# foubari/ratio_guided_Multimodal_FM

Measured on AMD Instinct MI355X. Metric: paired images/sec (MNIST32+SVHN, 100 Euler steps), higher is better.
Workload: dtype f32; 1 GPU; MNIST32 (1x32x32) + SVHN (3x32x32) pair, mc_feng guidance 0.5, 100 Euler steps, N_mc=256, batch 512 per GPU (BASELINE configs[2]; configs[3] at 8 GPUs); global_batch=512, parallelism=rows sharded over 1 rank(s); all_gather(MC set) + gather(outputs), step=one full sampling call (MC pre-phase + ratio + guided Euler loop + gather)

## Files before the change

### include/rgfm.h

```cpp
#ifndef RGFM_H_
#define RGFM_H_

#include <stddef.h>
#include <stdint.h>

#ifdef __cplusplus
extern "C" {
#endif

#define RGFM_ABI_VERSION 3

#define RGFM_OK 0
#define RGFM_EINVAL (-1)
#define RGFM_ENOMEM (-2)
#define RGFM_EHIP (-3)
#define RGFM_ENODEVICE (-4)

#define RGFM_MAX_LEVELS 4

typedef void* rgfm_stream_t;

typedef struct rgfm_unet_desc {
  int32_t in_channels;
  int32_t img_size;
// ... 1 lines not shown
  int32_t num_levels;
  int32_t channel_mult[RGFM_MAX_LEVELS];
  int32_t num_res_blocks;
} rgfm_unet_desc;

typedef struct rgfm_unet rgfm_unet;

int rgfm_unet_param_floats(const rgfm_unet_desc* desc, size_t* n_floats);

int rgfm_unet_create(const rgfm_unet_desc* desc, const float* params_dev, size_t n_floats,
                     rgfm_stream_t stream, rgfm_unet** out);
void rgfm_unet_destroy(rgfm_unet* h);

int rgfm_unet_workspace_bytes(const rgfm_unet* h, int batch, size_t* bytes);

int rgfm_unet_forward(rgfm_unet* h, const float* x, const float* t_dev, int t_count, float* v_out,
                      int batch, void* ws, size_t ws_bytes, rgfm_stream_t stream);

int rgfm_unet_set_trace(rgfm_unet* h, int enable);
int rgfm_unet_time_embedding(rgfm_unet* h, const float* t_dev, int t_count, float* emb_out, void* ws,
                             size_t ws_bytes, rgfm_stream_t stream);
int rgfm_unet_num_activations(const rgfm_unet* h, int* n);
int rgfm_unet_p_handovers(const rgfm_unet* h, int* blocks);
int rgfm_unet_wino_convs(const rgfm_unet* h, int* convs);
#define RGFM_ROUTE_HX2D 0
#define RGFM_ROUTE_HX2W 1
#define RGFM_ROUTE_HX2S 2
#define RGFM_ROUTE_HX2C 3
#define RGFM_ROUTE_HX2Q 4
#define RGFM_ROUTE_HX2P 5
#define RGFM_ROUTE_HX2 6
#define RGFM_ROUTE_BX3 7
#define RGFM_ROUTE_F32 8
#define RGFM_ROUTE_COUNT 9
#define RGFM_ROUTE_T2 9
#define RGFM_ROUTE_SLOTS 10
int rgfm_unet_conv_routes(const rgfm_unet* h, int* counts, int n);
int rgfm_unet_activation_shape(const rgfm_unet* h, int index, int* channels, int* height, int* width);
int rgfm_unet_read_activation(rgfm_unet* h, int index, int batch, const void* ws, float* out_dev,
                              rgfm_stream_t stream);

int rgfm_unet_train_workspace_bytes(const rgfm_unet* h, int batch, size_t* bytes);
int rgfm_unet_forward_train(rgfm_unet* h, const float* x, const float* t_dev, int t_count, float* v_out, int batch,
                            float p_drop, uint64_t seed, void* ws, size_t ws_bytes, rgfm_stream_t stream);
int rgfm_unet_backward(rgfm_unet* h, const float* dv, float* dx_out, float* dparams_out, int batch, void* ws,
                       size_t ws_bytes, rgfm_stream_t stream);
// ... 239 lines not shown
```

### ratio_guided_multimodal_fm_amd/_lib.py

```python
import ctypes
import os

_HERE = os.path.dirname(os.path.abspath(__file__))
LIB_PATH = os.environ.get("RGFM_LIB") or os.path.join(_HERE, "csrc", "librgfm_hip.so")
ABI_VERSION = 3

_lib = None

c_void_p, c_int, c_size_t, c_double = ctypes.c_void_p, ctypes.c_int, ctypes.c_size_t, ctypes.c_double
c_int32, c_int64, c_uint64, c_float = ctypes.c_int32, ctypes.c_int64, ctypes.c_uint64, ctypes.c_float
P = ctypes.POINTER


class UNetDesc(ctypes.Structure):
    _fields_ = [("in_channels", c_int32), ("img_size", c_int32), ("model_channels", c_int32),
                ("num_levels", c_int32), ("channel_mult", c_int32 * 4), ("num_res_blocks", c_int32)]


class RatioDesc(ctypes.Structure):
    _fields_ = [("kind", c_int32), ("feature_dim", c_int32), ("hidden_dim", c_int32),
                ("loss_type", c_int32)]


class RatioFlexDesc(ctypes.Structure):
    _fields_ = [("feature_dim", c_int32), ("hidden_dim", c_int32), ("loss_type", c_int32),
                ("x_channels", c_int32), ("y_channels", c_int32), ("x_size", c_int32), ("y_size", c_int32)]


class FmNetDesc(ctypes.Structure):
    _fields_ = [("img_channels", c_int32), ("feature_dim", c_int32), ("time_emb_dim", c_int32)]


class ClfDesc(ctypes.Structure):
    _fields_ = [("kind", c_int32)]


SIGNATURES = {
    "rgfm_unet_param_floats": (c_int, [P(UNetDesc), P(c_size_t)]),
    "rgfm_unet_create": (c_int, [P(UNetDesc), c_void_p, c_size_t, c_void_p, P(c_void_p)]),
    "rgfm_unet_destroy": (None, [c_void_p]),
    "rgfm_unet_workspace_bytes": (c_int, [c_void_p, c_int, P(c_size_t)]),
    "rgfm_unet_forward": (c_int, [c_void_p, c_void_p, c_void_p, c_int, c_void_p, c_int, c_void_p,
                                  c_size_t, c_void_p]),
    "rgfm_unet_set_trace": (c_int, [c_void_p, c_int]),
    "rgfm_unet_p_handovers": (c_int, [c_void_p, P(c_int)]),
    "rgfm_unet_wino_convs": (c_int, [c_void_p, P(c_int)]),
    "rgfm_unet_conv_routes": (c_int, [c_void_p, P(c_int), c_int]),
    "rgfm_unet_time_embedding": (c_int, [c_void_p, c_void_p, c_int, c_void_p, c_void_p, c_size_t, c_void_p]),
    "rgfm_unet_num_activations": (c_int, [c_void_p, P(c_int)]),
    "rgfm_unet_activation_shape": (c_int, [c_void_p, c_int, P(c_int), P(c_int), P(c_int)]),
    "rgfm_unet_read_activation": (c_int, [c_void_p, c_int, c_int, c_void_p, c_void_p, c_void_p]),
    "rgfm_unet_train_workspace_bytes": (c_int, [c_void_p, c_int, P(c_size_t)]),
    "rgfm_unet_forward_train": (c_int, [c_void_p, c_void_p, c_void_p, c_int, c_void_p, c_int, c_float, c_uint64,
                                        c_void_p, c_size_t, c_void_p]),
    "rgfm_unet_backward": (c_int, [c_void_p, c_void_p, c_void_p, c_void_p, c_int, c_void_p, c_size_t, c_void_p]),
    "rgfm_unet_vjp": (c_int, [c_void_p, c_void_p, c_void_p, c_int, c_void_p, c_size_t, c_void_p]),
    "rgfm_unet_divergence_workspace_bytes": (c_int, [c_void_p, c_int, P(c_size_t)]),
    "rgfm_unet_divergence": (c_int, [c_void_p, c_void_p, c_void_p, c_int, c_void_p, c_int, c_void_p, c_void_p, c_int,
                                     c_void_p, c_size_t, c_void_p]),
    "rgfm_unet_log_prob_workspace_bytes": (c_int, [c_void_p, c_int, c_int, c_int, P(c_size_t)]),
    "rgfm_unet_log_prob": (c_int, [c_void_p, c_void_p, c_void_p, c_int, c_int, c_int, c_void_p, c_void_p, c_int,
                                   c_void_p, c_size_t, c_void_p]),
    "rgfm_unet_dropout_mask": (c_int, [c_void_p, c_int, c_uint64, c_float, c_int, c_void_p]),
    "rgfm_unet_update_params": (c_int, [c_void_p, c_void_p, c_size_t, c_void_p]),
    "rgfm_ratio_param_floats": (c_int, [P(RatioDesc), P(c_size_t)]),
    "rgfm_ratio_create": (c_int, [P(RatioDesc), c_void_p, c_size_t, c_void_p, P(c_void_p)]),
    "rgfm_ratio_flex_param_floats": (c_int, [P(RatioFlexDesc), P(c_size_t)]),
    "rgfm_ratio_flex_create": (c_int, [P(RatioFlexDesc), c_void_p, c_size_t, c_void_p, P(c_void_p)]),
# ... 150 lines not shown
```

### ratio_guided_multimodal_fm_amd/csrc/api_unet.cpp

```cpp
#include "rgfm_host.h"

extern "C" int rgfm_unet_param_floats(const rgfm_unet_desc* desc, size_t* n_floats) {
  int rc = check_desc(desc);
  if (rc) return rc;
  if (!n_floats) return fail(RGFM_EINVAL, "null output");
  *n_floats = plan_unet(*desc, nullptr);
  return RGFM_OK;
}

static int pack_weights(rgfm_unet* h, hipStream_t s) {
  std::vector<HxImage*> images;
  std::vector<NormGate> gates;
  std::vector<ConvW*> res_convs;
  for (auto* v : {&h->enc, &h->mid, &h->dec})
    for (ResW& r : *v) {
      res_convs.push_back(&r.c1), res_convs.push_back(&r.c2);
      if (r.has_skip) res_convs.push_back(&r.sk);
      gates.push_back({r.n1w, r.n1b, r.cin, &r.c1.hx}), gates.push_back({r.n2w, r.n2b, r.cout, &r.c2.hx});
    }
  for (ConvW* w : res_convs) pack_one(h, *w, CONV_S1, s), images.push_back(&w->hx);
  for (ConvW& w : h->down) {
    pack_one(h, w, CONV_S2, s), images.push_back(&w.hx);
    launch_pack_conv_hx2(h->params + w.w_raw, h->packedh + w.hx9.off, h->hq + 4 * w.hx9.hq, w.cout, w.cin, 9, CONV_S1, s);
    images.push_back(&w.hx9);
// ... 161 lines not shown
  }
  for (int i = 0; i < 4; ++i) t.push_back({ch, S});
  for (int l = d.num_levels - 1; l >= 0; --l) {
    const int oc = h->mc * d.channel_mult[l];
    for (int i = 0; i < d.num_res_blocks + 1; ++i) {
      t.push_back({oc, S});
      t.push_back({oc, S});
      ch = oc;
    }
    if (l > 0) {
      S *= 2;
      t.push_back({ch, S});
    }
  }
  t.push_back({d.in_channels, S});
}
}

extern "C" int rgfm_unet_p_handovers(const rgfm_unet* h, int* blocks) {
  if (!h || !blocks) return fail(RGFM_EINVAL, "null argument");
  *blocks = h->p_handovers;
  return RGFM_OK;
}
extern "C" int rgfm_unet_wino_convs(const rgfm_unet* h, int* convs) {
  if (!h || !convs) return fail(RGFM_EINVAL, "null argument");
  *convs = h->wino_convs;
  return RGFM_OK;
}
extern "C" int rgfm_unet_conv_routes(const rgfm_unet* h, int* counts, int n) {
  if (!h || !counts || n < 0) return fail(RGFM_EINVAL, "null argument or negative count");
  for (int i = 0; i < n && i < RGFM_ROUTE_SLOTS; ++i) counts[i] = h->routes[i];
  return RGFM_OK;
}

extern "C" int rgfm_unet_num_activations(const rgfm_unet* h, int* n) {
  if (!h || !n) return fail(RGFM_EINVAL, "null argument");
  std::vector<std::pair<int, int>> t;
  act_table(h, t);
  *n = (int)t.size();
  return RGFM_OK;
}

extern "C" int rgfm_unet_activation_shape(const rgfm_unet* h, int index, int* channels, int* height, int* width) {
  if (!h) return fail(RGFM_EINVAL, "null handle");
  std::vector<std::pair<int, int>> t;
  act_table(h, t);
// ... 18 lines not shown
```

### ratio_guided_multimodal_fm_amd/csrc/rgfm_host.h

```cpp
#pragma once
#include "../../include/rgfm.h"

#include <hip/hip_runtime.h>

#include <algorithm>
#include <cmath>
#include <cstdarg>
#include <cstdio>
#include <cstdlib>
#include <cstring>
#include <string>
#include <vector>

#include "rgfm_kernels.h"

using namespace rgfm;

inline thread_local std::string g_err;

inline int fail(int code, const char* fmt, ...) {
  char buf[512];
  va_list ap;
  va_start(ap, fmt);
  vsnprintf(buf, sizeof(buf), fmt, ap);
// ... 178 lines not shown
  bool has_skip = false;
  int temb_off = 0;
};

inline int nt32_of(int cout) { return (cout % 64 == 0) ? 2 : 1; }

inline bool on_gfx950() {
  int dev = 0;
  if (hipGetDevice(&dev) != hipSuccess) return false;
  hipDeviceProp_t p;
  if (hipGetDeviceProperties(&p, dev) != hipSuccess) return false;
  return strncmp(p.gcnArchName, "gfx950", 6) == 0;
}

enum { CONV_ARITH_HX2 = 0, CONV_ARITH_BX3 = 1, CONV_ARITH_F32 = 2 };
struct Modes {
  int conv = CONV_ARITH_HX2;
  bool overlap = true, fuse_fin = true, gn_consumer = true;
  bool pipelined = true;
  bool quad = true;
  bool c8 = true;
  bool s2 = true;
  bool pfmt = true;
  bool wino = false;
  bool up_t2 = true;
  bool rev_hx2 = true;
  bool prephase = true;
  bool graph = false;
};
inline thread_local Modes g_modes;
inline void refresh_modes() {
  Modes m;
  const char* e = getenv("RGFM_CONV");
  if (e && strcmp(e, "bx3") == 0) m.conv = CONV_ARITH_BX3;
  else if (e && strcmp(e, "f32") == 0) m.conv = CONV_ARITH_F32;
  e = getenv("RGFM_OVERLAP");
  m.overlap = !(e && e[0] == '0');
  e = getenv("RGFM_FUSE_FIN");
  m.fuse_fin = !(e && e[0] == '0');
  e = getenv("RGFM_GN");
  m.gn_consumer = !(e && strcmp(e, "table") == 0);
  e = getenv("RGFM_HX2P");
  m.pipelined = !(e && e[0] == '0');
  e = getenv("RGFM_HX2Q");
  m.quad = !(e && e[0] == '0');
  e = getenv("RGFM_HX2S");
  m.s2 = !(e && e[0] == '0');
  e = getenv("RGFM_HX2C");
  m.c8 = !(e && e[0] == '0');
  e = getenv("RGFM_HX2D");
  m.pfmt = !(e && e[0] == '0');
  g_conv_tuning.hx2d_cut = e && e[0] == '1' ? 1 : (e && e[0] == '2' ? 2 : 3);
  e = getenv("RGFM_WINO");
  m.wino = e && e[0] == '1';
  e = getenv("RGFM_UP_T2");
  m.up_t2 = !(e && e[0] == '0');
  e = getenv("RGFM_REV_HX2");
  m.rev_hx2 = !(e && e[0] == '0');
  e = getenv("RGFM_GRAPH");
  m.graph = e && e[0] == '1';
  e = getenv("RGFM_PREPHASE_PRIO");
  m.prephase = !(e && e[0] == '0');
  g_modes = m;
  e = getenv("RGFM_WINO_W32");
  g_conv_tuning.wino_w32 = e ? atoi(e) : 0;
  g_conv_tuning.s2_f32 = getenv("RGFM_S2_F32") != nullptr;
  g_conv_tuning.f32_simple = getenv("RGFM_CONV_SIMPLE") != nullptr;
}

struct ModeScope {
  int saved;
  explicit ModeScope(int handle_mode) : saved(g_modes.conv) {
    if (handle_mode >= 0) g_modes.conv = handle_mode;
  }
  ~ModeScope() { g_modes.conv = saved; }
// ... 9 lines not shown
  hipEvent_t pre_pace = nullptr;
  hipStream_t main = nullptr;
  hipEvent_t main_fork = nullptr, main_join = nullptr;
  hipEvent_t graph_done = nullptr;
  std::vector<std::pair<hipGraphExec_t, hipGraph_t>> graphs;
};
inline DevState g_dev[MAX_DEVICES];

inline DevState* cur_dev() {
  int dev = 0;
  if (hipGetDevice(&dev) != hipSuccess || dev < 0 || dev >= MAX_DEVICES) return nullptr;
  return g_dev[dev].init ? &g_dev[dev] : nullptr;
}

inline int ensure_init() {
  if (!on_gfx950()) return fail(RGFM_ENODEVICE, "librgfm_hip needs a gfx950 (MI355X) device; none is current");
  int dev = 0;
  HIP_TRY(hipGetDevice(&dev));
  if (dev < 0 || dev >= MAX_DEVICES) return fail(RGFM_EINVAL, "device ordinal %d out of range (max %d)", dev, MAX_DEVICES - 1);
  DevState& d = g_dev[dev];
  if (!d.init) {
    int rc = guid_apply_init();
    for (const ConvKernel& k : CONV_KERNELS) rc |= k.init();
    if (rc != 0) return fail(RGFM_EHIP, "hipFuncSetAttribute(MaxDynamicSharedMemorySize) failed");
    hipDeviceProp_t p;
    if (hipGetDeviceProperties(&p, dev) == hipSuccess) d.num_cus = p.multiProcessorCount;
    const char* e = getenv("RGFM_HX2P_HALF");
    g_conv_tuning.hx2p_half = e ? atoi(e) : d.num_cus;
    HIP_TRY(hipStreamCreateWithFlags(&d.side, hipStreamNonBlocking));
    HIP_TRY(hipMalloc(&d.zeros, 256));
    HIP_TRY(hipMemset(d.zeros, 0, 256));
    HIP_TRY(hipEventCreateWithFlags(&d.fork, hipEventDisableTiming));
    HIP_TRY(hipEventCreateWithFlags(&d.join, hipEventDisableTiming));
    HIP_TRY(hipEventCreateWithFlags(&d.graph_done, hipEventDisableTiming));
    HIP_TRY(hipStreamCreateWithFlags(&d.main, hipStreamNonBlocking));
    HIP_TRY(hipEventCreateWithFlags(&d.main_fork, hipEventDisableTiming));
    HIP_TRY(hipEventCreateWithFlags(&d.main_join, hipEventDisableTiming));
    HIP_TRY(hipEventCreateWithFlags(&d.pre_pace, hipEventDisableTiming));
    d.init = true;
  }
  return RGFM_OK;
}

inline bool hx2w_pays(const ConvArgs& c) {
  return c.wpkw != nullptr && c.C0 + c.C1 >= 128 && (!g_conv_tuning.wino_w32 || c.g.W == 32);
}
// ... 114 lines not shown
  if (hipMemcpyAsync(host.data(), st.params, host.size() * sizeof(float), hipMemcpyDeviceToHost, s) != hipSuccess ||
      hipStreamSynchronize(s) != hipSuccess)
    return fail(RGFM_EHIP, "reading the parameters back failed");
  for (const NormGate& g : gates)
    if (!norm_params_ok(host, g.gamma, g.beta, g.C)) g.image->ok = false;
  return RGFM_OK;
}


struct rgfm_unet : WeightStore {
  rgfm_unet_desc d;
  float* freqs = nullptr;
  TimeLinear* lin_dev = nullptr;
  float* wtmp = nullptr;
  int mc = 0, temb = 0, nlin = 0, temb_total = 0;
  size_t te0w, te0b, te2w, te2b, icw, icb, onw, onb, ocw, ocb;
  size_t ocw_pk = 0;
  std::vector<ResW> enc, mid, dec;
  std::vector<ConvW> down, up;
  int final_ch = 0;
  bool trace = false;
  int wino_convs = 0;
  int p_handovers = 0;
  int routes[RGFM_ROUTE_SLOTS] = {};
  struct Act {
    float* data;
    int C, S;
    bool nchw;
  };
  std::vector<Act> acts;
};


inline size_t plan_unet(const rgfm_unet_desc& d, rgfm_unet* h) {
  Planner P;
  Cursor& c = P.raw;
  const int mc = d.model_channels, temb = 4 * mc;
  std::vector<ResW> enc, mid, dec;
  std::vector<ConvW> down, up;
  int temb_off = 0;
  auto res = [&](int cin, int cout) {
    ResW r;
    r.cin = cin, r.cout = cout;
    r.n1w = c.take(cin), r.n1b = c.take(cin);
    r.c1 = P.conv(cin, cout, 9);
    r.tw = c.take((size_t)cout * temb), r.tb = c.take(cout);
// ... 91 lines not shown
inline void fill_hx2(ConvArgs& c, const WeightStore& st, const ConvW& w, const ConvW* sk) {
  if (!w.hx.usable() || (sk && !sk->hx.usable())) return;
  c.wpkh = st.packedh + w.hx.off, c.hq = st.hq + 4 * w.hx.hq, c.range_flag = st.range_flag;
  if (w.hx9.usable()) c.wpkh9 = st.packedh + w.hx9.off;
  if (w.wino.usable() && !sk) c.wpkw = st.packedh + w.wino.off, c.hqw = st.hq + 4 * w.wino.hq;
  if (sk) c.wskiph = st.packedh + sk->hx.off, c.hq_skip = st.hq + 4 * sk->hx.hq;
}

inline double conv_flops(int B, int HW, int cout, int kprod) { return 2.0 * B * HW * (double)cout * kprod; }

inline bool up_parts_match(int S) {
  const TileGeom gl = make_geom(S, S), gf = make_geom(2 * S, 2 * S);
  if (gf.nparts != 4 * gl.nparts || gf.nparts > 16) return false;
  for (int p = 0; p < gf.nparts; ++p)
    if (geom_part_count(gf, p) != geom_part_count(gl, p % gl.nparts)) return false;
  return true;
}

struct PendingConv {
  bool valid = false;
  ConvArgs c{};
  int mode = 0;
  double flops = 0.0;
};

inline void flush_conv(PendingConv& p, hipStream_t s, int* routes = nullptr) {
  if (!p.valid) return;
  p.valid = false;
  ProfScope ps(RGFM_KCLASS_CONV_MFMA, p.flops, s);
  launch_conv(p.c, p.mode, s, routes);
}

inline bool try_fuse_finalize(PendingConv& p, const float* first_data, const float* stats1, int C1, const float* gamma,
                       const float* beta, float* ab, unsigned* counter) {
  if (!g_modes.fuse_fin || !p.valid || !counter || p.c.out != first_data || !p.c.stats_out) return false;
  if (p.c.pin0) return false;
  if ((p.c.Cout + C1) % 8 != 0 || p.c.Cout + C1 < 32 || p.c.Cout + C1 > 256) return false;
  if (p.c.g.nparts * (p.mode == CONV_T2 ? 4 : 1) > 16) return false;
  p.c.fin_ab = ab, p.c.fin_counter = counter, p.c.fin_expected = conv_fin_expected(p.c, p.mode);
  p.c.fin_stats1 = stats1, p.c.fin_C1 = C1, p.c.fin_gamma = gamma, p.c.fin_beta = beta;
  return true;
}

inline bool try_consumer_gn(ConvArgs& c, int mode, const float* stats0, const float* stats1, int nparts0, const TileGeom& gg,
                     const float* gamma, const float* beta) {
  c.gn_stats0 = stats0, c.gn_stats1 = stats1, c.gn_gamma = gamma, c.gn_beta = beta, c.gn_nparts0 = nparts0, c.gn_g = gg;
  bool ok = false;
  if (g_modes.gn_consumer) {
    if (g_modes.conv == CONV_ARITH_HX2 && conv_hx2_supported(c, mode)) ok = conv_hx2_gn_supported(c, mode);
    else if (g_modes.conv != CONV_ARITH_F32) ok = conv_bx3_gn_supported(c, mode);
  }
  if (!ok) c.gn_stats0 = c.gn_stats1 = c.gn_gamma = c.gn_beta = nullptr;
  return ok;
}

struct NormRef {
  size_t gamma, beta;
};
// ... 65 lines not shown
    c.out = o.data, c.stats_out = o.stats;
    c.B = B, c.Cout = w.cout;
    c.g = make_geom(So, So);
    c.halo_px = mode == CONV_S2 ? c.g.spt * (2 * c.g.th + 1) * (2 * c.g.W + 1) : c.g.spt * (c.g.th + 2) * (c.g.W + 2);
    const int kprod = 9 * w.cin + (res_mode == 2 ? sk->cin : 0);
    fill_hx2(c, *h, w, res_mode == 2 ? sk : nullptr);
    if (g_modes.conv == CONV_ARITH_HX2) c.range_flag = h->range_flag, c.small_check = raw_consumed ? 1 : 0;
    if (mode == CONV_UP2 && g_modes.conv == CONV_ARITH_HX2 && g_modes.up_t2 && w.t2.usable() && up_parts_match(a.S)) {
      ConvArgs ct = c;
      ct.g = make_geom(a.S, a.S);
      ct.halo_px = ct.g.spt * (ct.g.th + 2) * (ct.g.W + 2);
      ct.wpkh = h->packedh + w.t2.off, ct.hq = h->hq + 4 * w.t2.hq;
      if (conv_hx2_supported(ct, CONV_T2)) c = ct, mode = CONV_T2;
    }
    bool p_in = false;
    if (norm && a.p_valid && !b) {
      ConvArgs cp = c;
      DevState* ds = cur_dev();
      cp.pin0 = a.p, cp.zeros = ds ? ds->zeros : nullptr;
      if (pend.valid && pend.c.pout == a.p && conv_hx2d_supported(cp, mode)) {
        c = cp, p_in = true;
        h->p_handovers += 1;
        if (!h->trace) pend.c.out = nullptr, pend.c.stats_out = nullptr;
      } else if (pend.valid && pend.c.pout == a.p) {
        pend.c.pout = nullptr;
      }
    }
    if (norm && !p_in) {
      const TileGeom gg = make_geom(a.S, a.S);
      if (!try_consumer_gn(c, mode, a.stats, b ? b->stats : nullptr, gg.nparts, gg, h->params + norm->gamma,
                           h->params + norm->beta))
        c.ab = finalize(a, b, norm->gamma, norm->beta, ab_buf);
    }
    flush_conv(pend, s, h->routes);
    if (conv_route(c, mode) == RGFM_ROUTE_HX2W) h->wino_convs += 1;
    pend.valid = true, pend.c = c, pend.mode = mode;
    pend.flops = conv_flops(B, So * So, w.cout, kprod);
    return o;
  }
  Tensor resblock(const ResW& r, const Tensor& a, const Tensor* b) {
    const NormRef n1{r.n1w, r.n1b}, n2{r.n2w, r.n2b};
    Tensor h1 = conv(a, b, &n1, r.c1, CONV_S1, dry ? nullptr : temb_row + r.temb_off, 0, nullptr, nullptr, nullptr, false);
    if ((a.S == 8 || (a.S == 16 && r.cout == 64)) && r.cout % 64 == 0) {
      h1.p = ws->f((size_t)B * a.S * a.S * r.cout);
      if (!dry && pend.valid && pend.c.out == h1.data && r.c1.hx.ok && r.c2.hx.ok && (!r.has_skip || r.sk.hx.ok)) {
        pend.c.pout = h1.p, pend.c.pn_gamma = h->params + r.n2w, pend.c.pn_beta = h->params + r.n2b;
        if (p_producer_ok(pend.c, pend.mode)) h1.p_valid = true;
        else pend.c.pout = nullptr;
      }
    }
    record(h1);
    Tensor o = conv(h1, nullptr, &n2, r.c2, CONV_S1, nullptr, r.has_skip ? 2 : 1, &a, b, r.has_skip ? &r.sk : nullptr, true);
    record(o);
    return o;
  }

  int run(const float* x, float* v_out, float* x_state, float dt, const float* x_base = nullptr) {
    const rgfm_unet_desc& d = h->d;
    ModeScope mode_scope(h->conv_mode);
    if (!dry && h->trace) h->acts.clear();
    if (!dry) h->p_handovers = 0, h->wino_convs = 0, std::fill(h->routes, h->routes + RGFM_ROUTE_SLOTS, 0);
    int S = d.img_size;
    Tensor cur = new_tensor(h->mc, S);
    if (!dry) {
      ConvInArgs ci{};
      ci.x = x, ci.w = h->params + h->icw, ci.bias = h->params + h->icb;
      ci.out = cur.data, ci.stats_out = cur.stats, ci.B = B, ci.C0 = h->mc, ci.g = make_geom(S, S);
      ci.range_flag = h->range_flag, ci.small_check = g_modes.conv == CONV_ARITH_HX2 ? 1 : 0;
      const TileGeom g0 = make_geom(S, S);
      ProfScope p(d.in_channels == 1 ? RGFM_KCLASS_CONV_IN1 : RGFM_KCLASS_CONV_IN3,
                  4.0 * B * ((double)S * S * (d.in_channels + h->mc) + 2.0 * g0.nparts * h->mc), s);
      launch_conv_in(ci, d.in_channels, s);
    }
    record(cur);
    std::vector<Tensor> skips{cur};
    size_t e = 0;
    for (int l = 0; l < d.num_levels; ++l) {
      for (int r = 0; r < d.num_res_blocks; ++r) {
        cur = resblock(h->enc[e++], cur, nullptr);
        skips.push_back(cur);
      }
      if (l < d.num_levels - 1) {
        cur = conv(cur, nullptr, nullptr, h->down[l], CONV_S2, nullptr, 0, nullptr, nullptr, nullptr, true);
        record(cur);
// ... 208 lines not shown
```

### ratio_guided_multimodal_fm_amd/csrc/rgfm_kernels.h

```cpp
#pragma once
#include <hip/hip_runtime.h>
#include <stddef.h>
#include <stdint.h>

#include "../../include/rgfm.h"

namespace rgfm {

constexpr int KC = 16;
constexpr int LDP = 20;

struct TileGeom {
  int H, W, HW;
  int spt;
  int th;
  int tps;
  int nparts;
};

__host__ __device__ inline TileGeom make_geom(int H, int W) {
  TileGeom g;
  g.H = H;
  g.W = W;
  g.HW = H * W;
// ... 194 lines not shown
void launch_up2_as_deconv(const float* w, float* k, int Cout, int Cin, hipStream_t s);

bool conv_hx2p_supported(const ConvArgs& a, int mode);
int conv_hx2p_init();
bool launch_conv_hx2p(const ConvArgs& a, int mode, hipStream_t s);

bool conv_hx2q_supported(const ConvArgs& a, int mode);
int conv_hx2q_init();
bool launch_conv_hx2q(const ConvArgs& a, int mode, hipStream_t s);

bool conv_hx2s_supported(const ConvArgs& a, int mode);
int conv_hx2s_init();
bool launch_conv_hx2s(const ConvArgs& a, int mode, hipStream_t s);

bool conv_hx2c_supported(const ConvArgs& a, int mode);
int conv_hx2c_init();
bool launch_conv_hx2c(const ConvArgs& a, int mode, hipStream_t s);

bool conv_hx2d_supported(const ConvArgs& a, int mode);
int conv_hx2d_init();
bool launch_conv_hx2d(const ConvArgs& a, int mode, hipStream_t s);
void launch_hx_presplit(const float* in, const float* ab, void* pout, int B, int HW, int C, hipStream_t s);

bool conv_hx2w_supported(const ConvArgs& a, int mode);
int conv_hx2w_init();
bool launch_conv_hx2w(const ConvArgs& a, int mode, hipStream_t s);
void hx2_scale_launch(const float* w, size_t n, float* hq, hipStream_t s);
void launch_pack_conv_hx2w(const float* w, void* out, float* hq, float* tmp, int Cout, int Cin, hipStream_t s);

struct ConvKernel {
  const char* name;
  int (*init)();
  bool (*launch)(const ConvArgs& a, int mode, hipStream_t s);
};
inline constexpr ConvKernel CONV_KERNELS[RGFM_ROUTE_COUNT] = {
    {"hx2d", conv_hx2d_init, launch_conv_hx2d},
    {"hx2w", conv_hx2w_init, launch_conv_hx2w},
    {"hx2s", conv_hx2s_init, launch_conv_hx2s},
    {"hx2c", conv_hx2c_init, launch_conv_hx2c},
    {"hx2q", conv_hx2q_init, launch_conv_hx2q},
    {"hx2p", conv_hx2p_init, launch_conv_hx2p},
    {"hx2", conv_hx2_init, launch_conv_hx2},
    {"bx3", conv_bx3_init, launch_conv_bx3},
    {"f32", conv_mfma_init, launch_conv_mfma},
};
static_assert(RGFM_ROUTE_HX2D == 0 && RGFM_ROUTE_HX2W == 1 && RGFM_ROUTE_HX2S == 2 && RGFM_ROUTE_HX2C == 3 && RGFM_ROUTE_HX2Q == 4 &&
// ... 197 lines not shown
```

Baseline: 519.5 paired images/sec.

## Fuse both convs of 16x16 64-channel resblocks into one persistent kernel

Adds a new MFMA kernel that runs a resblock's first conv, its GroupNorm+SiLU handover into an in-LDS split-half image, and then the second conv with residual or skip path, all in one workgroup per image at 16x16 resolution. The host enables it by default (RGFM_RB16) whenever the pending producer conv and the next conv match the supported shape. The aim is to remove the intermediate activation round-trip through global memory and one kernel launch per eligible resblock. In exchange it uses a single 512-thread block per image with up to 160KB of LDS, which may limit occupancy and parallelism compared with the separate kernels.

```diff
diff --git a/include/rgfm.h b/include/rgfm.h
--- a/include/rgfm.h
+++ b/include/rgfm.h
@@ -47,6 +47,7 @@
                              size_t ws_bytes, rgfm_stream_t stream);
 int rgfm_unet_num_activations(const rgfm_unet* h, int* n);
 int rgfm_unet_p_handovers(const rgfm_unet* h, int* blocks);
+int rgfm_unet_rb16_blocks(const rgfm_unet* h, int* blocks);
 int rgfm_unet_wino_convs(const rgfm_unet* h, int* convs);
 #define RGFM_ROUTE_HX2D 0
 #define RGFM_ROUTE_HX2W 1
diff --git a/ratio_guided_multimodal_fm_amd/_lib.py b/ratio_guided_multimodal_fm_amd/_lib.py
--- a/ratio_guided_multimodal_fm_amd/_lib.py
+++ b/ratio_guided_multimodal_fm_amd/_lib.py
@@ -44,6 +44,7 @@
                                   c_size_t, c_void_p]),
     "rgfm_unet_set_trace": (c_int, [c_void_p, c_int]),
     "rgfm_unet_p_handovers": (c_int, [c_void_p, P(c_int)]),
+    "rgfm_unet_rb16_blocks": (c_int, [c_void_p, P(c_int)]),
     "rgfm_unet_wino_convs": (c_int, [c_void_p, P(c_int)]),
     "rgfm_unet_conv_routes": (c_int, [c_void_p, P(c_int), c_int]),
     "rgfm_unet_time_embedding": (c_int, [c_void_p, c_void_p, c_int, c_void_p, c_void_p, c_size_t, c_void_p]),
diff --git a/ratio_guided_multimodal_fm_amd/csrc/api_unet.cpp b/ratio_guided_multimodal_fm_amd/csrc/api_unet.cpp
--- a/ratio_guided_multimodal_fm_amd/csrc/api_unet.cpp
+++ b/ratio_guided_multimodal_fm_amd/csrc/api_unet.cpp
@@ -207,6 +207,11 @@
   *blocks = h->p_handovers;
   return RGFM_OK;
 }
+extern "C" int rgfm_unet_rb16_blocks(const rgfm_unet* h, int* blocks) {
+  if (!h || !blocks) return fail(RGFM_EINVAL, "null argument");
+  *blocks = h->rb16_blocks;
+  return RGFM_OK;
+}
 extern "C" int rgfm_unet_wino_convs(const rgfm_unet* h, int* convs) {
   if (!h || !convs) return fail(RGFM_EINVAL, "null argument");
   *convs = h->wino_convs;
diff --git a/ratio_guided_multimodal_fm_amd/csrc/conv_mfma_hx2r.hip b/ratio_guided_multimodal_fm_amd/csrc/conv_mfma_hx2r.hip
--- /dev/null
+++ b/ratio_guided_multimodal_fm_amd/csrc/conv_mfma_hx2r.hip
@@ -0,0 +1,497 @@
+#include <type_traits>
+
+#include "conv_hx2_common.h"
+
+namespace rgfm {
+
+namespace {
+constexpr int R_W = 16, R_WR = 18, R_PREC = R_WR * R_WR;
+constexpr int R_NTHR = 512, R_NW = 8;
+constexpr int R_TAPB = 64 * HRW;
+constexpr int R_UB = 3 * R_TAPB, R_CHB = 9 * R_TAPB;
+constexpr int R_PIMG = R_PREC * HRW;
+constexpr int R_ABYTES = (R_PREC + 1) * HRW;
+constexpr int R_REGION = 2 * R_CHB;
+constexpr int R_SX = R_NW * 32 * 2 * 4;
+static_assert(2 * R_ABYTES + 2 * R_UB <= R_REGION, "phase 1's buffers fit the region phase 2's weights take over");
+constexpr int R_MAXSKIP = 8;
+static_assert(R_MAXSKIP * R_TAPB <= R_CHB, "every skip chunk's tap of weights in one weight buffer");
+
+__device__ __forceinline__ float hx2r_p_emit(const f32x16& acc0, const f32x16& acc1, float sc, float sh, char* img, int seg, int l31, int hp) {
+  const bool odd = (l31 & 1) != 0;
+  const int slot = (l31 & 15) >> 3, inslot = ((l31 & 7) >> 1) * 4;
+  float m = 0.f;
+#pragma unroll
+  for (int mt = 0; mt < 2; ++mt)
+#pragma unroll
+    for (int r = 0; r < 16; r += 2) {
+      const f32x16& am = mt ? acc1 : acc0;
+      const float o0 = silu_scaled(fmaf(sc, am[r], sh)), o1 = silu_scaled(fmaf(sc, am[r + 1], sh));
+      const float recv = hx_swap1(odd ? o0 : o1);
+      const float lo = odd ? recv : o0, hi = odd ? o1 : recv;
+      m = hx_absmax3(lo, hi, m);
+      unsigned ph, pl;
+      hsplit2(lo, hi, ph, pl);
+      const int p = 64 * seg + 32 * mt + (r & 3) + 8 * (r >> 2) + 4 * hp + (odd ? 1 : 0);
+      const int y = p >> 4, x = p & 15;
+      const int rec = (y + 1) * R_WR + (x + 1);
+      const int off = rec * HRW + ((slot ^ ((x + 1) >> 1)) & 3) * 16 + inslot;
+      *reinterpret_cast<unsigned*>(img + off) = ph;
+      *reinterpret_cast<unsigned*>(img + (off ^ 32)) = pl;
+    }
+  return m;
+}
+}
+
+template <bool SKIP>
+__global__ __launch_bounds__(R_NTHR, 1) void conv_mfma_hx2r_kernel(const ConvArgs a, const ConvArgs a2) {
+  constexpr int W = R_W, WR = R_WR, NTHR = R_NTHR, NW = R_NW;
+  constexpr int TAPB = R_TAPB, UB = R_UB, CHB = R_CHB;
+  constexpr int NB = (UB / 16 + NTHR - 1) / NTHR;
+  constexpr int MAXIT = (R_PREC * 4 + NTHR - 1) / NTHR;
+  constexpr int MT_OFF = 2 * WR * HRW;
+  extern __shared__ __attribute__((aligned(16))) char smr[];
+  char* const sP = smr;
+  char* const sR = smr + 4 * R_PIMG;
+  char* const sB = sR + 2 * R_ABYTES;
+  float* const sx = reinterpret_cast<float*>(sR + R_REGION);
+  char* const sDesc = reinterpret_cast<char*>(sx) + R_SX;
+  float* const sTab = reinterpret_cast<float*>(sDesc + 256);
+
+  const int tid = threadIdx.x, lane = tid & 63, wave = tid >> 6;
+  const int grp = wave >> 2, seg = wave & 3;
+  const int l31 = lane & 31, hp = lane >> 5;
+  const int b0 = blockIdx.x;
+  const int n0 = grp * 32;
+  const int cin = a.C0 + a.C1;
+  const int nmain = cin / KC;
+  const int G = 3 * nmain;
+
+  {
+    const f32x4 z = {0.f, 0.f, 0.f, 0.f};
+    for (int i = tid; i < 4 * R_PIMG / 16; i += NTHR) *reinterpret_cast<f32x4*>(sP + i * 16) = z;
+  }
+
+  int aofs[3];
+  {
+    const int r = l31 / W, x = l31 % W;
+    const int arec = seg * 4 * WR + r * WR + x;
+#pragma unroll
+    for (int kx = 0; kx < 3; ++kx) aofs[kx] = (arec + kx) * HRW + ((hp ^ (((x + kx) >> 1) & 3)) & 3) * 16;
+  }
+  int bofs;
+  {
+    const int rec = n0 + l31;
+    bofs = rec * HRW + ((hp ^ (rec >> 2)) & 3) * 16;
+  }
+  const size_t pix0 = (size_t)b0 * (W * W) + seg * 64;
+  const int ch0 = n0 + l31;
+
+  const float qmain = a.hq[0];
+  const int gn_wsh = gn_waves_log2(cin >> 3);
+  const GnLane gn_lane(wave, lane, gn_wsh, cin >> 3);
+  float add0;
+  {
+    float v = a.bias[ch0];
+    if (a.temb) v += a.temb[((size_t)(a.temb_per_row ? b0 : 0) + (a.step_ptr ? (size_t)*a.step_ptr : 0)) * a.temb_stride + ch0];
+    add0 = v * qmain;
+  }
+  const int q4 = tid & 3;
+  int poff[MAXIT], adst[MAXIT], trow[MAXIT];
+#pragma unroll
+  for (int j = 0; j < MAXIT; ++j) {
+    const int it = tid + NTHR * j;
+    poff[j] = 0, adst[j] = R_PREC * HRW + (q4 >> 1) * 16 + (q4 & 1) * 8, trow[j] = (cin + 4 * q4) * 8;
+    if (it < R_PREC * 4) {
+      const int hpx = it >> 2;
+      const int hy = hpx / WR, hx = hpx - hy * WR;
+      const int y = hy - 1, x = hx - 1;
+      adst[j] = hpx * HRW + ((((q4 >> 1) ^ (hx >> 1)) & 3) * 16) + (q4 & 1) * 8;
+      if (y >= 0 && y < W && x >= 0 && x < W) {
+        poff[j] = (b0 * W + y) * W + x;
+        trow[j] = (4 * q4) * 8;
+      }
+    }
+  }
+  const char* const wpk = reinterpret_cast<const char*>(a.wpkh);
+  f32x4 ra[MAXIT], rb[NB];
+  int boff[NB];
+#pragma unroll
+  for (int j = 0; j < NB; ++j) {
+    const int it = tid + NTHR * j;
+    boff[j] = (it < UB / 16 ? it : it - UB / 16) * 16;
+  }
+  float hmax = 0.f;
+  auto chunk_desc = [&](int ch) { return *reinterpret_cast<const hx_u32x4*>(sDesc + ch * 16); };
+  auto issue_a = [&](const hx_u32x4& d, int j) {
+    const float* src = reinterpret_cast<const float*>(((unsigned long long)d.y << 32) | (unsigned long long)d.x);
+    ra[j] = *(const hx_gf32x4*)(src + (size_t)(__umul24((unsigned)poff[j], d.z) + (unsigned)(q4 * 4)));
+  };
+  auto table_a = [&](int ch, int j, f32x4& e0, f32x4& e1) {
+    const char* ep = reinterpret_cast<const char*>(sTab) + ch * (KC * 8) + trow[j];
+    e0 = *reinterpret_cast<const f32x4*>(ep);
+    e1 = *reinterpret_cast<const f32x4*>(ep + 16);
+  };
+  auto commit_a = [&](int ch, int j, const f32x4& e0, const f32x4& e1) {
+    f32x4 v = ra[j];
+    v.x = silu_scaled(fmaf(e0.x, v.x, e0.y));
+    v.y = silu_scaled(fmaf(e0.z, v.y, e0.w));
+    v.z = silu_scaled(fmaf(e1.x, v.z, e1.y));
+    v.w = silu_scaled(fmaf(e1.z, v.w, e1.w));
+    unsigned h0, l0, h1, l1;
+    hsplit2(v.x, v.y, h0, l0);
+    hsplit2(v.z, v.w, h1, l1);
+    hmax = hx_absmax3(v.x, v.y, hmax);
+    hmax = hx_absmax3(v.z, v.w, hmax);
+    const hx_u32x2 ph = {h0, h1}, pl = {l0, l1};
+    char* base = sR + (ch & 1) * R_ABYTES;
+    *reinterpret_cast<hx_u32x2*>(base + adst[j]) = ph;
+    *reinterpret_cast<hx_u32x2*>(base + (adst[j] ^ 32)) = pl;
+  };
+  auto issue_b = [&](int gg) {
+    const char* src = wpk + (size_t)gg * UB;
+#pragma unroll
+    for (int j = 0; j < NB; ++j) rb[j] = *(const hx_gf32x4*)(src + boff[j]);
+  };
+  auto commit_b = [&](int gg) {
+    char* dst = sB + (gg & 1) * UB;
+#pragma unroll
+    for (int j = 0; j < NB; ++j) *reinterpret_cast<f32x4*>(dst + boff[j]) = rb[j];
+  };
+
+  const unsigned long long in0_bits = reinterpret_cast<unsigned long long>(a.in0);
+  const hx_u32x4 d0 = {(unsigned)in0_bits, (unsigned)(in0_bits >> 32), (unsigned)a.C0, 0u};
+#pragma unroll
+  for (int j = 0; j < MAXIT; ++j) issue_a(d0, j);
+  issue_b(0);
+  if (gn_lane.row < 1) gn_table_row(a, gn_lane, b0, true, sTab, HX_SA);
+  hx_tab_zero_row(sTab, 1, cin, NTHR);
+  hx_store_chunk_desc(a, sDesc, nmain, nmain);
+  __syncthreads();
+  {
+#pragma unroll
+    for (int j = 0; j < MAXIT; ++j) {
+      f32x4 e0, e1;
+      table_a(0, j, e0, e1);
+      commit_a(0, j, e0, e1);
+    }
+    commit_b(0);
+    const hx_u32x4 d1 = chunk_desc(1);
+#pragma unroll
+    for (int j = 0; j < MAXIT; ++j) issue_a(d1, j);
+    issue_b(1);
+  }
+  f32x16 acc[2][1];
+#pragma unroll
+  for (int mt = 0; mt < 2; ++mt)
+#pragma unroll
+    for (int r = 0; r < 16; ++r) acc[mt][0][r] = add0;
+  __syncthreads();
+
+  typedef HxFrag<> Frag;
+#define HX2R_SEG() __builtin_amdgcn_sched_barrier(0x0002 | 0x0004 | 0x0010 | 0x0400)
+  int gidx = 0;
+  auto unit_fast = [&](int c, auto u_tag) {
+    constexpr int U = decltype(u_tag)::value;
+    const char* sArow = sR + (c & 1) * R_ABYTES + U * WR * HRW;
+    const char* sBu = sB + (gidx & 1) * UB;
+    char* sBn = sB + ((gidx + 1) & 1) * UB;
+    const char* wsrc = wpk + (size_t)(gidx + 2) * UB;
+    Frag f0, f1;
+    f0.load(sArow, aofs[0], MT_OFF, sBu, bofs);
+    const int c2 = c + 2 < nmain ? c + 2 : nmain - 1;
+    const hx_u32x4 dn = chunk_desc(c2);
+    f32x4 e0, e1;
+    table_a(c + 1, U, e0, e1);
+    HX2R_SEG();
+    f1.load(sArow, aofs[1], MT_OFF, sBu + TAPB, bofs);
+    f0.mma(acc);
+    HX2R_SEG();
+#pragma unroll
+    for (int j = 0; j < NB; ++j) *reinterpret_cast<f32x4*>(sBn + boff[j]) = rb[j];
+    commit_a(c + 1, U, e0, e1);
+    issue_a(dn, U);
+#pragma unroll
+    for (int j = 0; j < NB; ++j) rb[j] = *(const hx_gf32x4*)(wsrc + boff[j]);
+    f0.load(sArow, aofs[2], MT_OFF, sBu + 2 * TAPB, bofs);
+    f1.mma(acc);
+    HX2R_SEG();
+    f0.mma(acc);
+    __syncthreads();
+    ++gidx;
+  };
+  auto unit_tail = [&](int c, auto u_tag) {
+    constexpr int U = decltype(u_tag)::value;
+    const char* sArow = sR + (c & 1) * R_ABYTES + U * WR * HRW;
+    const char* sBu = sB + (gidx & 1) * UB;
+    Frag f0, f1;
+    f0.load(sArow, aofs[0], MT_OFF, sBu, bofs);
+    HX2R_SEG();
+    f1.load(sArow, aofs[1], MT_OFF, sBu + TAPB, bofs);
+    f0.mma(acc);
+    HX2R_SEG();
+    if (U < 2) {
+      char* sBn = sB + ((gidx + 1) & 1) * UB;
+#pragma unroll
+      for (int j = 0; j < NB; ++j) *reinterpret_cast<f32x4*>(sBn + boff[j]) = rb[j];
+    }
+    if (U < 1) {
+      const char* wsrc = wpk + (size_t)(gidx + 2) * UB;
+#pragma unroll
+      for (int j = 0; j < NB; ++j) rb[j] = *(const hx_gf32x4*)(wsrc + boff[j]);
+    }
+    f0.load(sArow, aofs[2], MT_OFF, sBu + 2 * TAPB, bofs);
+    f1.mma(acc);
+    HX2R_SEG();
+    f0.mma(acc);
+    __syncthreads();
+    ++gidx;
+  };
+#undef HX2R_SEG
+  using U0 = std::integral_constant<int, 0>;
+  using U1 = std::integral_constant<int, 1>;
+  using U2 = std::integral_constant<int, 2>;
+  {
+    int c0 = 0;
+#pragma unroll 1
+    for (; c0 < nmain - 1; ++c0) {
+      unit_fast(c0, U0{});
+      unit_fast(c0, U1{});
+      unit_fast(c0, U2{});
+    }
+    unit_tail(c0, U0{});
+    unit_tail(c0, U1{});
+    unit_tail(c0, U2{});
+  }
+  (void)G;
+
+  const int nskip = SKIP ? (a2.R0 + a2.R1) / KC : 0;
+  constexpr int nmain2 = 4;
+  const int wave_s = __builtin_amdgcn_readfirstlane(wave);
+  const unsigned sR_lds = (unsigned)(size_t)sR;
+  const char* const wpk2 = reinterpret_cast<const char*>(a2.wpkh);
+  const char* const wsk2 = reinterpret_cast<const char*>(SKIP ? a2.wskiph : a2.wpkh);
+  constexpr int PPT = TAPB / 1024, NPW = 5;
+  auto dma = [&](const char* gsrc, unsigned dst) {
+    unsigned keep;
+    asm volatile("s_mov_b32 %0, m0\n\ts_mov_b32 m0, %2\n\ts_nop 0\n\tglobal_load_lds_dwordx4 %1, off\n\ts_mov_b32 m0, %0"
+                 : "=&s"(keep)
+                 : "v"(gsrc), "s"(dst)
+                 : "memory");
+  };
+  auto wdma1 = [&](int c, int j) {
+    const int pq = wave_s + NW * j;
+    const int pc = pq < 9 * PPT ? pq : pq - 9 * PPT;
+    dma(wpk2 + (size_t)c * CHB + pc * 1024 + lane * 16, sR_lds + (unsigned)((c & 1) * CHB + pc * 1024));
+  };
+  auto sdma1 = [&](int j) {
+    const int pq = wave_s + NW * j;
+    if (pq < nskip * PPT) dma(wsk2 + (size_t)pq * 1024 + lane * 16, sR_lds + (unsigned)(pq * 1024));
+  };
+  auto wdma = [&](int c) {
+#pragma unroll
+    for (int j = 0; j < NPW; ++j) wdma1(c, j);
+  };
+  wdma(0);
+
+  constexpr int NIS = SKIP ? (W * W * 4) / NTHR : 1;
+  unsigned spix[NIS];
+  int sdst[NIS];
+  if (SKIP) {
+#pragma unroll
+    for (int j = 0; j < NIS; ++j) {
+      const int it = tid + NTHR * j, px = it >> 2;
+      const int y = px / W, x = px - y * W;
+      const int rec = (y + 1) * WR + (x + 1);
+      sdst[j] = rec * HRW + ((((q4 >> 1) ^ ((x + 1) >> 1)) & 3) * 16) + (q4 & 1) * 8;
+      spix[j] = (unsigned)(b0 * (W * W) + px);
+    }
+  }
+  f32x4 rs0[NIS], rs1[NIS], rs2[NIS], rs3[NIS];
+  float hmax2 = 0.f;
+  auto sissue = [&](f32x4 (&rr)[NIS], int k) {
+    const int c = k * KC;
+    const bool first = c < a2.R0;
+    const float* src = first ? a2.res0 + c : a2.res1 + (c - a2.R0);
+    const unsigned cs = (unsigned)(first ? a2.R0 : a2.R1);
+#pragma unroll
+    for (int j = 0; j < NIS; ++j) rr[j] = *(const hx_gf32x4*)(src + (size_t)(__umul24(spix[j], cs) + (unsigned)(q4 * 4)));
+  };
+  auto scommit = [&](const f32x4 (&rr)[NIS], int k) {
+    char* base = sP + (k & 3) * R_PIMG;
+#pragma unroll
+    for (int j = 0; j < NIS; ++j) {
+      const float sa = HX_SA;
+      const f32x4 v = rr[j];
+      f32x4 o;
+      o.x = v.x * sa, o.y = v.y * sa, o.z = v.z * sa, o.w = v.w * sa;
+      unsigned h0, l0, h1, l1;
+      hsplit2(o.x, o.y, h0, l0);
+      hsplit2(o.z, o.w, h1, l1);
+      hmax2 = hx_absmax3(o.x, o.y, hmax2);
+      hmax2 = hx_absmax3(o.z, o.w, hmax2);
+      const hx_u32x2 ph = {h0, h1}, pl = {l0, l1};
+      *reinterpret_cast<hx_u32x2*>(base + sdst[j]) = ph;
+      *reinterpret_cast<hx_u32x2*>(base + (sdst[j] ^ 32)) = pl;
+    }
+  };
+  if (SKIP) {
+    sissue(rs0, 0);
+    if (nskip > 1) sissue(rs1, 1);
+    if (nskip > 2) sissue(rs2, 2);
+    if (nskip > 3) sissue(rs3, 3);
+  }
+  const float qmain2 = a2.hq[0];
+  f32x16 acc2[2][1];
+  hx_acc_init<SKIP>(acc2, a2, b0, pix0, ch0, hp, qmain2);
+
+  {
+    const float qinv = a.hq[1];
+#pragma unroll
+    for (int mt = 0; mt < 2; ++mt) acc[mt][0] = acc[mt][0] * qinv;
+    if (!(hmax < HX_BIG)) atomicOr(a.range_flag, 1u);
+  }
+  {
+    const float gam = a.pn_gamma[ch0], bet = a.pn_beta[ch0];
+    float mean, m2;
+    hx_stats64(acc, 0, mean, m2);
+    if (hp == 0) {
+      float2 v;
+      v.x = mean, v.y = m2;
+      *reinterpret_cast<float2*>(sx + (wave * 32 + l31) * 2) = v;
+    }
+    __syncthreads();
+    double s1 = 0.0, s2 = 0.0;
+#pragma unroll
+    for (int sg = 0; sg < 4; ++sg) {
+      const float2 v = *reinterpret_cast<const float2*>(sx + ((wave - seg + sg) * 32 + l31) * 2);
+      s1 += 64.0 * (double)v.x;
+      s2 += (double)v.y + 64.0 * (double)v.x * (double)v.x;
+    }
+    float sc, sh;
+    hx_group_affine_s(s1, s2, 256.0, 8, gam, bet, sc, sh);
+    const float pm = hx2r_p_emit(acc[0][0], acc[1][0], sc, sh, sP + (ch0 >> 4) * R_PIMG, seg, l31, hp);
+    if (!(pm < HX_BIG)) atomicOr(a.range_flag, 1u);
+  }
+
+  auto ldf = [&](Frag& f, const char* sArow, const char* sBt, int o0) { f.load(sArow, o0, MT_OFF, sBt, bofs); };
+  auto iteration = [&](f32x4 (&rr)[NIS], int c) {
+    asm volatile("s_waitcnt vmcnt(0)" ::: "memory");
+    __syncthreads();
+    const char* sBc = sR + (c & 1) * CHB;
+    const bool nxt = c + 1 < nmain2;
+    auto dma_slot = [&](int t) {
+#pragma unroll
+      for (int k = 2 * t; k < 2 * t + 2; ++k) {
+        if (k < NPW && nxt) wdma1(c + 1, k);
+        if (SKIP && k < 4 && !nxt) sdma1(k);
+      }
+    };
+    const char* sAc = sP + c * R_PIMG;
+    Frag f0, f1;
+#define HX2R_LDF(F, T) ldf(F, sAc + ((T) / 3) * WR * HRW, sBc + (T) * TAPB, aofs[(T) % 3])
+#define HX2R_STEP(FN, FC, T)               \
+  do {                                     \
+      HX2R_LDF(FN, (T) + 1);                 \
+      __builtin_amdgcn_sched_barrier(0);     \
+      dma_slot(T);                           \
+      FC.mma(acc2);                          \
+      __builtin_amdgcn_sched_barrier(0);     \
+  } while (0)
+    HX2R_LDF(f0, 0);
+    HX2R_STEP(f1, f0, 0);
+    HX2R_STEP(f0, f1, 1);
+    HX2R_STEP(f1, f0, 2);
+    HX2R_STEP(f0, f1, 3);
+    HX2R_STEP(f1, f0, 4);
+    HX2R_STEP(f0, f1, 5);
+    HX2R_STEP(f1, f0, 6);
+    HX2R_STEP(f0, f1, 7);
+    f0.mma(acc2);
+#undef HX2R_STEP
+#undef HX2R_LDF
+    if (SKIP && c >= 1 && c - 1 < nskip) {
+      scommit(rr, c - 1);
+      if (c + 3 < nskip) sissue(rr, c + 3);
+    }
+  };
+  iteration(rs0, 0);
+  iteration(rs0, 1);
+  iteration(rs1, 2);
+  iteration(rs2, 3);
+  if (SKIP) {
+    {
+      const float rs = a2.hq_skip[0] * a2.hq[1];
+#pragma unroll
+      for (int mt = 0; mt < 2; ++mt) acc2[mt][0] = acc2[mt][0] * rs;
+    }
+    auto position = [&](f32x4 (&rr)[NIS], int k) {
+      if (k == 0) asm volatile("s_waitcnt vmcnt(0)" ::: "memory");
+      __syncthreads();
+      Frag f;
+      ldf(f, sP + (k & 3) * R_PIMG + WR * HRW, sR + k * TAPB, aofs[1]);
+      f.mma(acc2);
+      if (k + 3 < nskip) {
+        scommit(rr, k + 3);
+        if (k + 7 < nskip) sissue(rr, k + 7);
+      }
+    };
+    if (0 < nskip) position(rs3, 0);
+    if (1 < nskip) position(rs0, 1);
+    if (2 < nskip) position(rs1, 2);
+    if (3 < nskip) position(rs2, 3);
+    if (4 < nskip) position(rs3, 4);
+    if (5 < nskip) position(rs0, 5);
+    if (6 < nskip) position(rs1, 6);
+    if (7 < nskip) position(rs2, 7);
+  }
+  if (SKIP && !(hmax2 < HX_BIG)) atomicOr(a2.range_flag, 1u);
+
+  {
+    const float qinv = SKIP ? a2.hq_skip[1] : a2.hq[1];
+#pragma unroll
+    for (int mt = 0; mt < 2; ++mt) acc2[mt][0] = acc2[mt][0] * qinv;
+  }
+  if (a2.small_check && a2.range_flag) hx_small_scan(a2.range_flag, acc2);
+#pragma unroll
+  for (int mt = 0; mt < 2; ++mt)
+#pragma unroll
+    for (int r = 0; r < 16; ++r) a2.out[(pix0 + hx_acc_pixel(mt, r, hp)) * 64 + ch0] = acc2[mt][0][r];
+  if (a2.stats_out) {
+    float mean, m2;
+    hx_stats64(acc2, 0, mean, m2);
+    if (hp == 0) store_stats(a2, a2.stats_out + (((size_t)b0 * a2.g.nparts + seg) * 64 + ch0) * 2, mean, m2);
+  }
+}
+
+static size_t hx2r_lds_bytes(const ConvArgs& c1) {
+  return (size_t)4 * R_PIMG + R_REGION + R_SX + 256 + (size_t)2 * (c1.C0 + c1.C1) * 2 * sizeof(float);
+}
+
+bool conv_hx2r_supported(const ConvArgs& c1, const ConvArgs& c2) {
+  const TileGeom& g = c1.g;
+  if (!(g.W == 16 && g.H == 16 && g.spt == 1 && g.tps == 1) || c1.Hin != 16 || c1.Win != 16) return false;
+  if (c1.Cout != 64 || c2.Cout != 64 || c2.C0 != 64 || c2.C1 != 0 || c2.g.W != 16 || c2.g.H != 16) return false;
+  if (!c1.gn_stats0 || c1.ab || c1.res_mode != 0 || c1.ep_scale || c1.fin_ab || c1.in_amax || c1.out || c1.stats_out) return false;
+  if (!c1.pout || !c1.pn_gamma || !c1.pn_beta || !c1.wpkh || !c1.hq || !c1.range_flag) return false;
+  const int cin = c1.C0 + c1.C1;
+  if (cin % KC != 0 || c1.C0 % KC != 0 || cin < 2 * KC || cin > 256) return false;
+  if (c2.res_mode != 1 && c2.res_mode != 2) return false;
+  if (c2.ep_scale || c2.fin_ab || !c2.out || !c2.wpkh || !c2.hq || !c2.range_flag || c2.B != c1.B) return false;
+  if (c2.res_mode == 2 && (c2.R0 + c2.R1) / KC > R_MAXSKIP) return false;
+  return hx2r_lds_bytes(c1) <= 160 * 1024;
+}
+
+int conv_hx2r_init() {
+  int rc = raise_lds_limit(&conv_mfma_hx2r_kernel<false>, 160 * 1024);
+  rc |= raise_lds_limit(&conv_mfma_hx2r_kernel<true>, 160 * 1024);
+  return rc;
+}
+
+void launch_conv_hx2r(const ConvArgs& c1, const ConvArgs& c2, hipStream_t s) {
+  const size_t lds = hx2r_lds_bytes(c1);
+  if (c2.res_mode == 2) hipLaunchKernelGGL(conv_mfma_hx2r_kernel<true>, dim3(c1.B), dim3(R_NTHR), lds, s, c1, c2);
+  else hipLaunchKernelGGL(conv_mfma_hx2r_kernel<false>, dim3(c1.B), dim3(R_NTHR), lds, s, c1, c2);
+}
+
+}
diff --git a/ratio_guided_multimodal_fm_amd/csrc/rgfm_host.h b/ratio_guided_multimodal_fm_amd/csrc/rgfm_host.h
--- a/ratio_guided_multimodal_fm_amd/csrc/rgfm_host.h
+++ b/ratio_guided_multimodal_fm_amd/csrc/rgfm_host.h
@@ -224,6 +224,7 @@
   bool c8 = true;
   bool s2 = true;
   bool pfmt = true;
+  bool rb16 = true;
   bool wino = false;
   bool up_t2 = true;
   bool rev_hx2 = true;
@@ -253,6 +254,8 @@
   e = getenv("RGFM_HX2D");
   m.pfmt = !(e && e[0] == '0');
   g_conv_tuning.hx2d_cut = e && e[0] == '1' ? 1 : (e && e[0] == '2' ? 2 : 3);
+  e = getenv("RGFM_RB16");
+  m.rb16 = !(e && e[0] == '0');
   e = getenv("RGFM_WINO");
   m.wino = e && e[0] == '1';
   e = getenv("RGFM_UP_T2");
@@ -308,6 +311,7 @@
   if (!d.init) {
     int rc = guid_apply_init();
     for (const ConvKernel& k : CONV_KERNELS) rc |= k.init();
+    rc |= conv_hx2r_init();
     if (rc != 0) return fail(RGFM_EHIP, "hipFuncSetAttribute(MaxDynamicSharedMemorySize) failed");
     hipDeviceProp_t p;
     if (hipGetDeviceProperties(&p, dev) == hipSuccess) d.num_cus = p.multiProcessorCount;
@@ -468,6 +472,7 @@
   bool trace = false;
   int wino_convs = 0;
   int p_handovers = 0;
+  int rb16_blocks = 0;
   int routes[RGFM_ROUTE_SLOTS] = {};
   struct Act {
     float* data;
@@ -605,18 +610,26 @@
   ConvArgs c{};
   int mode = 0;
   double flops = 0.0;
+  bool fused = false;
+  ConvArgs c2{};
 };
 
 inline void flush_conv(PendingConv& p, hipStream_t s, int* routes = nullptr) {
   if (!p.valid) return;
   p.valid = false;
   ProfScope ps(RGFM_KCLASS_CONV_MFMA, p.flops, s);
+  if (p.fused) {
+    p.fused = false;
+    if (routes) routes[RGFM_ROUTE_HX2P] += 1, routes[RGFM_ROUTE_HX2D] += 1;
+    launch_conv_hx2r(p.c, p.c2, s);
+    return;
+  }
   launch_conv(p.c, p.mode, s, routes);
 }
 
 inline bool try_fuse_finalize(PendingConv& p, const float* first_data, const float* stats1, int C1, const float* gamma,
                        const float* beta, float* ab, unsigned* counter) {
-  if (!g_modes.fuse_fin || !p.valid || !counter || p.c.out != first_data || !p.c.stats_out) return false;
+  if (!g_modes.fuse_fin || !p.valid || p.fused || !counter || p.c.out != first_data || !p.c.stats_out) return false;
   if (p.c.pin0) return false;
   if ((p.c.Cout + C1) % 8 != 0 || p.c.Cout + C1 < 32 || p.c.Cout + C1 > 256) return false;
   if (p.c.g.nparts * (p.mode == CONV_T2 ? 4 : 1) > 16) return false;
@@ -728,6 +741,12 @@
         c = cp, p_in = true;
         h->p_handovers += 1;
         if (!h->trace) pend.c.out = nullptr, pend.c.stats_out = nullptr;
+        if (!h->trace && g_modes.rb16 && conv_hx2r_supported(pend.c, c)) {
+          pend.fused = true, pend.c2 = c;
+          pend.flops += conv_flops(B, So * So, w.cout, kprod);
+          h->rb16_blocks += 1;
+          return o;
+        }
       } else if (pend.valid && pend.c.pout == a.p) {
         pend.c.pout = nullptr;
       }
@@ -740,7 +759,7 @@
     }
     flush_conv(pend, s, h->routes);
     if (conv_route(c, mode) == RGFM_ROUTE_HX2W) h->wino_convs += 1;
-    pend.valid = true, pend.c = c, pend.mode = mode;
+    pend.valid = true, pend.fused = false, pend.c = c, pend.mode = mode;
     pend.flops = conv_flops(B, So * So, w.cout, kprod);
     return o;
   }
@@ -765,7 +784,7 @@
     const rgfm_unet_desc& d = h->d;
     ModeScope mode_scope(h->conv_mode);
     if (!dry && h->trace) h->acts.clear();
-    if (!dry) h->p_handovers = 0, h->wino_convs = 0, std::fill(h->routes, h->routes + RGFM_ROUTE_SLOTS, 0);
+    if (!dry) h->p_handovers = 0, h->rb16_blocks = 0, h->wino_convs = 0, std::fill(h->routes, h->routes + RGFM_ROUTE_SLOTS, 0);
     int S = d.img_size;
     Tensor cur = new_tensor(h->mc, S);
     if (!dry) {
diff --git a/ratio_guided_multimodal_fm_amd/csrc/rgfm_kernels.h b/ratio_guided_multimodal_fm_amd/csrc/rgfm_kernels.h
--- a/ratio_guided_multimodal_fm_amd/csrc/rgfm_kernels.h
+++ b/ratio_guided_multimodal_fm_amd/csrc/rgfm_kernels.h
@@ -240,6 +240,10 @@
 bool launch_conv_hx2d(const ConvArgs& a, int mode, hipStream_t s);
 void launch_hx_presplit(const float* in, const float* ab, void* pout, int B, int HW, int C, hipStream_t s);
 
+bool conv_hx2r_supported(const ConvArgs& c1, const ConvArgs& c2);
+int conv_hx2r_init();
+void launch_conv_hx2r(const ConvArgs& c1, const ConvArgs& c2, hipStream_t s);
+
 bool conv_hx2w_supported(const ConvArgs& a, int mode);
 int conv_hx2w_init();
 bool launch_conv_hx2w(const ConvArgs& a, int mode, hipStream_t s);
```

New measurement: 516.9 paired images/sec. No clear change (-0.5%).
